# gregc-91/GPU-Raytracing

Hardware: AMD Instinct MI355X
Metric: Mrays/s at 1920x1080 primary rays + BVH build ms, 1M-tri scene (higher is better)
Workload: dtype f32; 1 GPU; grid_mesh(G=708, seed=1) = 1002528 triangles, 1920x1080, 1 spp, camera A (top-down), render_type 0; LBVH replicated per GPU; parallelism=row-bands x1, 8 frames in flight on 8 HIP streams

## Files before the change

### gpu-raytracing_amd/csrc/rt_traverse.hpp

```cpp
#pragma once

#include "rt_device.hpp"
#include "rt_math.h"

namespace rt {

constexpr int kStackLds = 16;
constexpr int kStackMax = 64;
constexpr uint32_t kPrefetchMinPrims = 8u << 20;
#ifndef RT_TRACE_WAVES
#define RT_TRACE_WAVES 4
#endif
constexpr int kTraceWaves = RT_TRACE_WAVES;
#ifndef RT_TRACE_MIN_WAVES
#define RT_TRACE_MIN_WAVES 7
#endif
#ifndef RT_TRACE_LEAN_EXTRA
#define RT_TRACE_LEAN_EXTRA 1
#endif
#ifndef RT_TRACE_PF_WAVES
#define RT_TRACE_PF_WAVES 5
#endif

#ifndef RT_TRACE_UNIFORM_MAX
#define RT_TRACE_UNIFORM_MAX 0
#endif
constexpr int kUniformMax = RT_TRACE_UNIFORM_MAX;
#ifndef RT_TRACE_UNIFORM_STICKY
#define RT_TRACE_UNIFORM_STICKY 1
#endif
constexpr bool kUniformSticky = RT_TRACE_UNIFORM_STICKY != 0;
#ifndef RT_TRACE_PAIR_BARRIER
#define RT_TRACE_PAIR_BARRIER 0
#endif
#ifndef RT_TRACE_LEAF_WIDE
#define RT_TRACE_LEAF_WIDE 1
#endif

constexpr int kParkNum = 8, kParkDen = 1;

#ifndef RT_TRACE_XCD_CHUNK
#define RT_TRACE_XCD_CHUNK 8
#endif
__device__ __forceinline__ uint32_t xcd_chunk_block(uint32_t bid, uint32_t nb)
{
    constexpr uint32_t kXcdChunk = RT_TRACE_XCD_CHUNK;
    const uint32_t full = nb / (8u * kXcdChunk) * (8u * kXcdChunk);
    const uint32_t xcd = bid & 7u, loc = bid >> 3;
    return bid < full ? (loc / kXcdChunk) * (8u * kXcdChunk) + xcd * kXcdChunk + (loc % kXcdChunk) : bid;
}

typedef __attribute__((address_space(3))) uint32_t lds_u32;

struct Ray {
    float ox, oy, oz, dx, dy, dz, ix, iy, iz, tmin, tmax;
};
struct Hit {
    uint32_t primitive_id, tri_id;
    float bu, bv;
};

struct NoFilter {
    static constexpr bool active = false;
};

template <class Filter = NoFilter>
__device__ __forceinline__ bool intersect_tri(float v0x, float v0y, float v0z, float v1x, float v1y, float v1z,
                                              float v2x, float v2y, float v2z, Ray& r, Hit& h, uint32_t tri_id,
                                              uint32_t prim_id, Filter flt = Filter())
{
    const float epsilon = 0.000000001f;
    const float e1x = v1x - v0x, e1y = v1y - v0y, e1z = v1z - v0z;
    const float e2x = v2x - v0x, e2y = v2y - v0y, e2z = v2z - v0z;
    const float hx = r.dy * e2z - r.dz * e2y, hy = r.dz * e2x - r.dx * e2z, hz = r.dx * e2y - r.dy * e2x;
    const float a = e1x * hx + e1y * hy + e1z * hz;
    if (a > -epsilon && a < epsilon) return false;
    const float f = 1.0f / a;
    const float sx = r.ox - v0x, sy = r.oy - v0y, sz = r.oz - v0z;
    const float u = f * (sx * hx + sy * hy + sz * hz);
    if (u < 0.0f || u > 1.0f) return false;
    const float qx = sy * e1z - sz * e1y, qy = sz * e1x - sx * e1z, qz = sx * e1y - sy * e1x;
    const float v = f * (r.dx * qx + r.dy * qy + r.dz * qz);
    if (v < 0.0f || (u + v) > 1.0f) return false;
    const float t = f * (e2x * qx + e2y * qy + e2z * qz);
    if (t < r.tmin || t > r.tmax) return false;
    if constexpr (Filter::active) {
        if (!flt.keep(a, prim_id)) return false;
    }
    r.tmax = t;
    h.primitive_id = prim_id;
    h.tri_id = tri_id;
    h.bu = u;
    h.bv = v;
    return true;
}

enum : uint32_t { PH_STEP = 0, PH_LEAF0 = 1, PH_LEAF1 = 2, PH_DONE = 3 };
constexpr uint32_t kNoNear = 0xFFFFFFFFu;

typedef uint32_t SpillArray[kStackMax - kStackLds];

struct Trav {
    lds_u32* lds;
    uint32_t* spill;
    int sp;
    uint32_t cur;
    uint32_t near_e;
    float near_d;
    uint32_t phase;
    uint32_t leaf;
    float f1, k1;
    uint32_t e1;
    uint32_t t1;
    uint32_t box_tests, tri_tests;
    uint4 pf0, pf1, pf2, pf3;

    __device__ __forceinline__ void push(uint32_t e)
    {
        if (sp < kStackLds) lds[sp * 64] = e;
        else if (sp < kStackMax) spill[sp - kStackLds] = e;
        sp = min(sp + 1, kStackMax);
    }
    __device__ __forceinline__ void inner_hit(bool in, uint32_t e, float front)
    {
        const bool closer = (front < near_d) | ((front == near_d) & ((e & kIndexMask) > (near_e & kIndexMask)));
        if (in & (near_e != kNoNear)) push(closer ? near_e : e);
        const bool take = in & closer;
        near_e = take ? e : near_e;
        near_d = take ? front : near_d;
    }
    __device__ __forceinline__ void advance()
    {
        const uint32_t cnt = cur >> 29;
        if (cnt > 2) { cur = ((cur & kIndexMask) + 2) | ((cnt - 2) << 29); return; }
        const bool keep = (near_e != kNoNear) & (sp < kStackMax);
        if (keep) cur = near_e;
        else if (sp == 0) phase = PH_DONE;
        else { --sp; cur = sp < kStackLds ? lds[sp * 64] : spill[sp - kStackLds]; }
        near_e = kNoNear;
        near_d = __builtin_inff();
    }
    __device__ __forceinline__ void second_slot(float tmin, float tmax)
    {
        const bool valid = t1 != RT_CHILD_NONE;
        const bool hit = valid & (k1 >= f1) & (f1 <= tmax) & (k1 >= tmin);
        box_tests += valid ? 1u : 0u;
        const bool is_leaf = hit & (t1 == RT_CHILD_TRI);
        inner_hit(hit & !is_leaf, e1, f1);
        if (is_leaf) { leaf = e1; phase = PH_LEAF1; }
    }
};

__device__ __forceinline__ void slab(const uint4& a, const uint4& b, const Ray& r, float& front, float& back)
{
    typedef float v2f __attribute__((ext_vector_type(2)));
    const v2f o2 = {r.ox, r.oy}, i2 = {r.ix, r.iy};
    const v2f lo = {__uint_as_float(a.x), __uint_as_float(a.y)}, hi = {__uint_as_float(b.x), __uint_as_float(b.y)};
    const v2f t1 = (lo - o2) * i2, t2 = (hi - o2) * i2;
    const float t1z = (__uint_as_float(a.z) - r.oz) * r.iz, t2z = (__uint_as_float(b.z) - r.oz) * r.iz;
    front = fmaxf(fmaxf(fminf(t1.x, t2.x), fminf(t1.y, t2.y)), fminf(t1z, t2z));
    back = fminf(fminf(fmaxf(t1.x, t2.x), fmaxf(t1.y, t2.y)), fmaxf(t1z, t2z));
}

template <bool PF, class Params>
__device__ __forceinline__ void prefetch_pair(const Params& p, Trav& t)
{
    if constexpr (PF) {
        if (t.phase == PH_STEP) {
            const uint4* np = reinterpret_cast<const uint4*>(p.nodes + (t.cur & kIndexMask));
            const int o1 = (t.cur >> 29) > 1 ? 2 : 0;
            t.pf0 = np[0]; t.pf1 = np[1]; t.pf2 = np[o1]; t.pf3 = np[o1 + 1];
        }
    }
}

template <bool PF, class Params>
__device__ __forceinline__ void box_step_on(const Params& p, const Ray& r, Trav& t, bool two, const uint4& a0, const uint4& b0,
                                            const uint4& a1, const uint4& b1)
{
    float f0, k0;
    slab(a0, b0, r, f0, k0);
    slab(a1, b1, r, t.f1, t.k1);
    t.e1 = (b1.w & kIndexMask) | (a1.w & ~kIndexMask);
    t.t1 = two ? (b1.w >> 29) : (uint32_t)RT_CHILD_NONE;
    const uint32_t type0 = b0.w >> 29;
    const uint32_t e0 = (b0.w & kIndexMask) | (a0.w & ~kIndexMask);
    const bool valid0 = type0 != RT_CHILD_NONE;
    const bool hit0 = valid0 & (k0 >= f0) & (f0 <= r.tmax) & (k0 >= r.tmin);
    t.box_tests += valid0 ? 1u : 0u;
    const bool leaf0 = hit0 & (type0 == RT_CHILD_TRI);
    t.inner_hit(hit0 & !leaf0, e0, f0);
    if (leaf0) { t.leaf = e0; t.phase = PH_LEAF0; }
    else {
        t.second_slot(r.tmin, r.tmax);
        if (t.phase == PH_STEP) { t.advance(); prefetch_pair<PF>(p, t); }
    }
}

template <bool PF, class Params>
__device__ __forceinline__ void box_step(const Params& p, const Ray& r, Trav& t)
{
    const uint32_t cnt = t.cur >> 29;
    const uint4* np = reinterpret_cast<const uint4*>(p.nodes + (t.cur & kIndexMask));
#ifdef RT_EXP_BOX_PAD
#pragma unroll
    for (int q = 0; q < RT_EXP_BOX_PAD; q++) asm volatile("v_mov_b32 %0, %0" : "+v"(t.box_tests));
#endif
    const bool two = cnt > 1;
    const int o1 = two ? 2 : 0;
    uint4 a0, b0, a1, b1;
    if constexpr (PF) { a0 = t.pf0; b0 = t.pf1; a1 = t.pf2; b1 = t.pf3; }
    else {
        a0 = np[0]; b0 = np[1]; a1 = np[o1]; b1 = np[o1 + 1];
#if RT_TRACE_PAIR_BARRIER
        __builtin_amdgcn_sched_barrier(0);
#endif
    }
    box_step_on<PF>(p, r, t, two, a0, b0, a1, b1);
}

typedef uint32_t u32x4 __attribute__((ext_vector_type(4)));
typedef const __attribute__((address_space(4))) u32x4* const_u4_ptr;
template <class Params>
__device__ __forceinline__ void box_step_shared(const Params& p, const Ray& r, Trav& t, uint32_t c)
{
    c = (uint32_t)__builtin_amdgcn_readfirstlane((int)c);
    const const_u4_ptr np = (const_u4_ptr)(uintptr_t)(p.nodes + (c & kIndexMask));
    const bool two = (c >> 29) > 1;
    const int o1 = two ? 2 : 0;
    const u32x4 a0 = np[0], b0 = np[1], a1 = np[o1], b1 = np[o1 + 1];
    box_step_on<false>(p, r, t, two, make_uint4(a0.x, a0.y, a0.z, a0.w), make_uint4(b0.x, b0.y, b0.z, b0.w),
                       make_uint4(a1.x, a1.y, a1.z, a1.w), make_uint4(b1.x, b1.y, b1.z, b1.w));
}

template <bool PF, class Params>
__device__ __forceinline__ bool box_step_wave(const Params& p, const Ray& r, Trav& t, uint64_t st)
{
    if constexpr (!PF && kUniformMax > 0) {
        constexpr int K = kUniformMax > 0 ? kUniformMax : 1;
        uint32_t cs[K];
        uint64_t ms[K];
        uint64_t rest = st;
#pragma unroll
        for (int k = 0; k < kUniformMax; k++) {
            cs[k] = 0; ms[k] = 0;
            if (rest) {
                cs[k] = (uint32_t)__builtin_amdgcn_readlane((int)t.cur, __ffsll((unsigned long long)rest) - 1);
                ms[k] = __builtin_amdgcn_ballot_w64(t.phase == PH_STEP && t.cur == cs[k]);
                rest &= ~ms[k];
            }
        }
        if (rest == 0) {
#pragma unroll
            for (int k = 0; k < kUniformMax; k++)
                if (ms[k]) { if (t.phase == PH_STEP && t.cur == cs[k]) box_step_shared(p, r, t, cs[k]); }
            return true;
        }
    }
    if (t.phase == PH_STEP) box_step<PF>(p, r, t);
    return false;
}

template <bool PF, bool ANY = false, class Params, class Filter = NoFilter>
__device__ __forceinline__ bool trace_ray(const Params& p, Ray& r, Hit& h, Trav& t, bool active, uint32_t* steps,
                                          Filter flt = Filter())
{
    t.sp = 0;
    t.cur = (p.root & kIndexMask) | (p.count << 29);
    t.near_e = kNoNear;
    t.near_d = __builtin_inff();
    t.phase = (active && p.count > 0) ? PH_STEP : PH_DONE;
    t.box_tests = 0;
    t.tri_tests = 0;
    t.t1 = 0;
    t.e1 = 0;
    t.f1 = t.k1 = 0.0f;
    t.leaf = 0;
    prefetch_pair<PF>(p, t);
    bool tri_hit = false;
    uint32_t nbox = 0, nleaf = 0;
    bool shared = true;
#ifdef RT_EXP_UNIFORM_STATS
    uint32_t ustat[4] = {0, 0, 0, 0};
#endif

    while (true) {
        uint64_t stepping, parked;
        while (true) {
            stepping = __builtin_amdgcn_ballot_w64(t.phase == PH_STEP);
            parked = __builtin_amdgcn_ballot_w64((t.phase - 1u) < 2u);
            if (stepping == 0 || __popcll(stepping) * p.park_den < __popcll(parked) * p.park_num) break;
            nbox += 2;
#ifdef RT_EXP_UNIFORM_STATS
            {
                uint64_t rest = stepping;
                int distinct = 0;
                while (rest && distinct < 5) {
                    const int l0 = __ffsll((unsigned long long)rest) - 1;
                    const uint32_t c0 = (uint32_t)__builtin_amdgcn_readlane((int)t.cur, l0);
                    rest &= ~__builtin_amdgcn_ballot_w64(t.phase == PH_STEP && t.cur == c0);
                    distinct++;
                }
                ustat[distinct <= 1 ? 0 : (distinct == 2 ? 1 : (distinct <= 4 ? 2 : 3))]++;
            }
#endif
            if constexpr (!PF && kUniformMax > 0) {
                if (!kUniformSticky || shared) {
                    shared = box_step_wave<PF>(p, r, t, stepping);
                    const uint64_t again = __builtin_amdgcn_ballot_w64(t.phase == PH_STEP);
                    if (again) shared = box_step_wave<PF>(p, r, t, again);
                    continue;
                }
            }
            if (t.phase == PH_STEP) box_step<PF>(p, r, t);
            if (t.phase == PH_STEP) box_step<PF>(p, r, t);
        }
        if ((stepping | parked) == 0) break;
        nleaf++;
        if ((t.phase - 1u) < 2u) {
            t.tri_tests++;
            const uint32_t li = t.leaf & kIndexMask;
            const uint4* tp = reinterpret_cast<const uint4*>(p.leaves + li);
            uint4 l0 = tp[0], l1 = tp[1], l2 = tp[2], l3 = tp[3];
#if RT_TRACE_LEAF_WIDE
            asm volatile("" : "+v"(l0.x), "+v"(l0.y), "+v"(l0.z), "+v"(l0.w), "+v"(l1.x), "+v"(l1.y), "+v"(l1.z), "+v"(l1.w),
                              "+v"(l2.x), "+v"(l2.y), "+v"(l2.z), "+v"(l2.w), "+v"(l3.x), "+v"(l3.y), "+v"(l3.z), "+v"(l3.w));
#endif
            bool hit_tri = intersect_tri(__uint_as_float(l0.x), __uint_as_float(l0.y), __uint_as_float(l0.z),
                                         __uint_as_float(l1.x), __uint_as_float(l1.y), __uint_as_float(l1.z),
                                         __uint_as_float(l2.x), __uint_as_float(l2.y), __uint_as_float(l2.z),
                                         r, h, li << 1, l0.w, flt);
            if ((t.leaf >> 29) > 0 && (l3.x != l2.x || l3.y != l2.y || l3.z != l2.z))
                hit_tri |= intersect_tri(__uint_as_float(l2.x), __uint_as_float(l2.y), __uint_as_float(l2.z),
                                         __uint_as_float(l1.x), __uint_as_float(l1.y), __uint_as_float(l1.z),
                                         __uint_as_float(l3.x), __uint_as_float(l3.y), __uint_as_float(l3.z),
                                         r, h, (li << 1) + 1, l1.w, flt);
            tri_hit |= hit_tri;
            if (ANY && hit_tri) {
                t.phase = PH_DONE;
            } else {
                const bool was_first = t.phase == PH_LEAF0;
                t.phase = PH_STEP;
                if (was_first) t.second_slot(r.tmin, r.tmax);
                if (t.phase == PH_STEP) { t.advance(); prefetch_pair<PF>(p, t); }
            }
        }
    }
#ifdef RT_EXP_UNIFORM_STATS
    steps[0] += ustat[RT_EXP_UNIFORM_STATS == 1 ? 0 : 2];
    steps[1] += ustat[RT_EXP_UNIFORM_STATS == 1 ? 1 : 3];
    (void)nbox; (void)nleaf;
#elif !defined(RT_TRACE_NO_STEPS)
    steps[0] += nbox;
    steps[1] += nleaf;
#endif
    return tri_hit;
}

__device__ __forceinline__ void camera_ray(const rt_camera& cam, uint32_t w, uint32_t h, uint32_t x, uint32_t y, float ox,
                                           float oy, Ray& r)
{
    const float ndcx = 2 * (((float)x + ox) / (float)w) - 1;
    const float ndcy = 2 * (((float)y + oy) / (float)h) - 1;
    const float px = (ndcx * cam.u.x + ndcy * cam.v.x) + 1.0f * cam.w.x;
    const float py = (ndcx * cam.u.y + ndcy * cam.v.y) + 1.0f * cam.w.y;
    const float pz = (ndcx * cam.u.z + ndcy * cam.v.z) + 1.0f * cam.w.z;
    const float inv_len = 1.0f / sqrtf(px * px + py * py + pz * pz);
    r.dx = px * inv_len; r.dy = py * inv_len; r.dz = pz * inv_len;
    r.ox = cam.position.x; r.oy = cam.position.y; r.oz = cam.position.z;
    r.tmin = 0.00001f;
    r.tmax = cam.max_depth;
}

__device__ __forceinline__ void subpixel_offset(uint32_t s, uint32_t spp, float& ox, float& oy)
{
    const uint32_t side = spp == 4 ? 2u : 4u;
    ox = ((float)(s % side) + 0.5f) / (float)side;
    oy = ((float)((s / side) % side) + 0.5f) / (float)side;
}

}
```

### gpu-raytracing_amd/csrc/trace_kernel.hip

```cpp
#include <cstdio>
#include <cstdlib>

#include "rt_device.hpp"
#include "rt_launch.hpp"
#include "rt_math.h"
#include "rt_shade.hpp"
#include "rt_traverse.hpp"

namespace rt {

#ifdef RT_TRACE_TUNING
constexpr int kRenderDebugBoxCount = 100;
#else
constexpr int kRenderDebugBoxCount = -1;
#endif
#ifndef RT_TRACE_TILE_2X2
#define RT_TRACE_TILE_2X2 0
#endif


constexpr uint32_t kCtrSlots = 256, kCtrSub = 16;
struct alignas(64) CtrSlot {
    unsigned long long part[kCtrSub][8];
    unsigned long long top, pad[7];
};
__device__ CtrSlot g_ctr[kCtrSlots];

struct TraceParams {
    const rt_node* nodes;
    const rt_triangle_pair* leaves;
    const rt_attributes* attributes;
    const rt_material* materials;
    const rt_texture* textures;
    const rt_camera* camera;
    float light[3];
    uint32_t root, count, num_materials, num_textures;
    uint8_t* rgba8;
    uint32_t w, h, y0, y1, spp;
    unsigned long long* counters;
    uint32_t tiles_x, num_tiles;
    uint32_t strip_tiles, strip_first, strip_stride;
    int park_num, park_den;
    uint32_t ctr_slot;
};



template <int RENDER, bool PF>
__device__ __forceinline__ void shade_sample(const TraceParams& p, const rt_camera& cam, uint32_t x, uint32_t y,
                                             float ox, float oy, Trav& t, bool active, uint32_t& box_acc,
                                             uint32_t& tri_acc, uint32_t* steps, float& R, float& G, float& B, float& A)
{
    const float max_depth = cam.max_depth;
    Ray r;
    camera_ray(cam, p.w, p.h, x, y, ox, oy, r);
    r.ix = 1.0f / r.dx; r.iy = 1.0f / r.dy; r.iz = 1.0f / r.dz;
    Hit h = {0u, 0u, 0.f, 0.f};
    const bool hit = trace_ray<PF>(p, r, h, t, active, steps);
    const uint32_t box_tests = t.box_tests, tri_tests = t.tri_tests;
    box_acc += box_tests;
    tri_acc += tri_tests;
    const float depth = hit ? r.tmax : 0.0f;
    R = G = B = 0;
    A = 255.0f;

    if (RENDER == RT_RENDER_DEPTH) {
        R = G = B = fminf(1.0f, depth / max_depth) * 255;
        return;
    }
    if (RENDER == RT_RENDER_BOXTESTS) {
        G = B = fminf(box_tests / 180.0f, 1.0f) * 255;
        return;
    }
    if (RENDER == kRenderDebugBoxCount) {
        R = __uint_as_float(box_tests);
        return;
    }
    if (RENDER == RT_RENDER_TRIANGLE_TESTS) {
        const float g = fminf(tri_tests / 32.0f, 1.0f);
        R = g * 100; G = g * 255; B = g * 100;
        return;
    }
    const bool lit = active && hit;
    const bool fetch = active && (hit || RENDER == RT_RENDER_LODS);
    rt_material mat = {};
    Surface s = {};
    int material_id = 0;
    if (fetch) {
        const rt_triangle_pair* pair = p.leaves + (h.tri_id >> 1);
        const bool second = h.tri_id & 1;
        const uint32_t rot = second ? pair->rotations[1] : pair->rotations[0];
        const rt_attributes* at = p.attributes + h.primitive_id;
        const int i0 = rot == 1 ? 2 : (rot == 2 ? 1 : 0);
        const int i1 = rot == 1 ? 0 : (rot == 2 ? 2 : 1);
        const int i2 = rot == 1 ? 1 : (rot == 2 ? 0 : 2);
        material_id = at->material_id;
        mat = p.materials[(uint32_t)material_id < p.num_materials ? (uint32_t)material_id : 0u];
        if ((uint32_t)mat.texture >= p.num_textures) mat.texture = -1;
        if ((uint32_t)mat.bump >= p.num_textures) mat.bump = -1;
        if ((uint32_t)mat.disp >= p.num_textures) mat.disp = -1;
        const rt_float3 n0 = at->normal[i0], n1 = at->normal[i1], n2 = at->normal[i2];
        s.n[0] = v3(n0.x, n0.y, n0.z); s.n[1] = v3(n1.x, n1.y, n1.z); s.n[2] = v3(n2.x, n2.y, n2.z);
        if (render_uses_surface(RENDER)) {
            s.uv[0][0] = at->uv[i0][0]; s.uv[0][1] = at->uv[i0][1];
            s.uv[1][0] = at->uv[i1][0]; s.uv[1][1] = at->uv[i1][1];
            s.uv[2][0] = at->uv[i2][0]; s.uv[2][1] = at->uv[i2][1];
            const rt_float3 a = second ? pair->v2 : pair->v0, b = pair->v1, c = second ? pair->v3 : pair->v2;
            s.tri[0] = v3(a.x, a.y, a.z); s.tri[1] = v3(b.x, b.y, b.z); s.tri[2] = v3(c.x, c.y, c.z);
        }
    }
    const float spread = 2.0f / p.w;
    if (RENDER == RT_RENDER_LODS) {
        if (!active) return;
        if (mat.texture != -1 && hit) {
            const float lod = compute_lod(r, h, spread, s, p.textures[mat.texture]);
            R = G = B = A = (float)(((uint32_t)((int)lod * 20)) & 255u);
        } else {
            R = 255; G = 0; B = 255;
        }
        return;
    }
    if (RENDER == RT_RENDER_MATERIAL_ID) {
        if (lit) hsv_to_rgb255((float)material_id / p.num_materials, 1.0f, 1.0f, R, G, B);
        return;
    }
    if (RENDER == RT_RENDER_TEXTURE) {
        if (!lit) return;
        if (mat.texture != -1) {
            const rt_texture& tex = p.textures[mat.texture];
            const float lod = compute_lod(r, h, spread, s, tex);
            const U8x4 c = trilinear_sample(tex, interp_uv(s, h.bu, h.bv), lod);
            R = (float)c.c[0]; G = (float)c.c[1]; B = (float)c.c[2]; A = (float)c.c[3];
        } else {
            R = mat.diffuse.x * 255; G = mat.diffuse.y * 255; B = mat.diffuse.z * 255;
        }
        return;
    }
    constexpr bool use_textures = RENDER == RT_RENDER_TEXTURE_LIT || RENDER == RT_RENDER_TEXTURE_LIT_SHADOWS;
    constexpr bool use_bump = use_textures;
    constexpr bool use_shadows = RENDER == RT_RENDER_TEXTURE_LIT_SHADOWS;
    const float hx = r.ox + r.dx * r.tmax, hy = r.oy + r.dy * r.tmax, hz = r.oz + r.dz * r.tmax;
    float lx = p.light[0] - hx, ly = p.light[1] - hy, lz = p.light[2] - hz;
    const float to_light = sqrtf(lx * lx + ly * ly + lz * lz);
    const float linv = 1.0f / to_light;
    lx *= linv; ly *= linv; lz *= linv;
    bool shadowed = false;
    if (use_shadows) {
        Ray sr;
        sr.ox = hx; sr.oy = hy; sr.oz = hz;
        sr.dx = lx; sr.dy = ly; sr.dz = lz;
        sr.ix = 1.0f / lx; sr.iy = 1.0f / ly; sr.iz = 1.0f / lz;
        sr.tmin = 0.001f;
        sr.tmax = to_light;
        Hit sh = {0u, 0u, 0.f, 0.f};
        shadowed = trace_ray<PF>(p, sr, sh, t, lit, steps);
    }
    if (!lit) return;
    const float w0 = 1 - h.bu - h.bv;
    V3 n = vadd(vadd(vscale(s.n[0], w0), vscale(s.n[1], h.bu)), vscale(s.n[2], h.bv));
    if (use_bump && mat.disp != -1) {
        const rt_texture& disp = p.textures[mat.disp];
        const float lod = compute_lod(r, h, spread, s, disp);
        V3 tbn[3];
        tangent_matrix(s, tbn);
        const U8x4 smp = trilinear_sample(disp, interp_uv(s, h.bu, h.bv), lod);
        n = v3((float)smp.c[0] / 255.0f, (float)smp.c[1] / 255.0f, (float)smp.c[2] / 255.0f);
        n = vnormalize(v3(n.x * 2.0f - 1.0f, n.y * 2.0f - 1.0f, n.z * 2.0f - 1.0f));
        n = vnormalize(v3(vdot(tbn[0], n), vdot(tbn[1], n), vdot(tbn[2], n)));
    } else if (use_bump && mat.bump != -1) {
        const rt_texture& bump = p.textures[mat.bump];
        const float lod = compute_lod(r, h, spread, s, bump);
        V3 tbn[3];
        tangent_matrix(s, tbn);
        n = bump2normal(bump, tbn, interp_uv(s, h.bu, h.bv), lod);
    }
    const float nx = n.x, ny = n.y, nz = n.z;
    const float lcx = 1.0f, lcy = 0.9f, lcz = 0.8f;
    float dterm = 1.0f * fmaxf(nx * lx + ny * ly + nz * lz, 0.0f);
    const float nlx = -lx, nly = -ly, nlz = -lz;
    const float ndl = nx * nlx + ny * nly + nz * nlz;
    const float rx = nlx - (nx * 2.0f) * ndl, ry = nly - (ny * 2.0f) * ndl, rz = nlz - (nz * 2.0f) * ndl;
    const double sb = fmax((double)((-r.dx) * rx + (-r.dy) * ry + (-r.dz) * rz), 0.0);
    float sp = (float)(1.0f * rt_pow_d(sb, (double)mat.specular_exp));
    float odx = mat.diffuse.x, ody = mat.diffuse.y, odz = mat.diffuse.z;
    if (use_textures && mat.texture != -1) {
        const rt_texture& tex = p.textures[mat.texture];
        const float lod = compute_lod(r, h, spread, s, tex);
        const U8x4 smp = bilinear_sample(tex, interp_uv(s, h.bu, h.bv), (int)lod);
        odx = (float)smp.c[0] / 255; ody = (float)smp.c[1] / 255; odz = (float)smp.c[2] / 255;
    }
    float dfx = lcx * dterm, dfy = lcy * dterm, dfz = lcz * dterm;
    float spx = lcx * sp, spy = lcy * sp, spz = lcz * sp;
    if (shadowed) { dfx = dfy = dfz = 0.0f; spx = spy = spz = 0.0f; }
    const float cr = (dfx * odx + (lcx * 0.2f) * mat.ambient.x) + spx * mat.specular.x;
    const float cg = (dfy * ody + (lcy * 0.2f) * mat.ambient.y) + spy * mat.specular.y;
    const float cb = (dfz * odz + (lcz * 0.2f) * mat.ambient.z) + spz * mat.specular.z;
    R = clampf(cr, 0.0f, 1.0f) * 255;
    G = clampf(cg, 0.0f, 1.0f) * 255;
    B = clampf(cb, 0.0f, 1.0f) * 255;
}

template <int RENDER, bool PF>
__global__ __launch_bounds__(kTraceWaves * 64, PF ? RT_TRACE_PF_WAVES : ((RENDER <= 2 || RENDER == kRenderDebugBoxCount) ? RT_TRACE_MIN_WAVES + RT_TRACE_LEAN_EXTRA : RT_TRACE_MIN_WAVES))
void trace_kernel(TraceParams p)
{
    __shared__ uint32_t stack_lds[kTraceWaves][kStackLds][64];
    __shared__ unsigned long long csum[4];
    __shared__ uint32_t carrive;
    const int lane = threadIdx.x & 63, wave = threadIdx.x >> 6;
    if (p.counters) {
        if (threadIdx.x < 4) csum[threadIdx.x] = 0ull;
        if (threadIdx.x == 4) carrive = 0u;
        __syncthreads();
    }

    const uint32_t vb = xcd_chunk_block(blockIdx.x, gridDim.x);
#if RT_TRACE_TILE_2X2
    const uint32_t blocks_x = (p.tiles_x + 1) / 2;
    const uint32_t tx = (vb % blocks_x) * 2 + (wave & 1), ty = (vb / blocks_x) * 2 + (wave >> 1);
    const uint32_t tile = tx < p.tiles_x ? ty * p.tiles_x + tx : p.num_tiles;
#else
    const uint32_t tile = vb * kTraceWaves + wave;
    const uint32_t tx = tile % p.tiles_x, ty = tile / p.tiles_x;
#endif

    const uint32_t lx = (lane & 1) | ((lane >> 1) & 2) | ((lane >> 2) & 4);
    const uint32_t ly = ((lane >> 1) & 1) | ((lane >> 2) & 2) | ((lane >> 3) & 4);
    const uint32_t x = tx * 8 + lx;
    uint32_t y = p.y0 + ty * 8 + ly, out_y = y;
    if (p.strip_tiles) {
        const uint32_t strip = p.strip_first + (ty / p.strip_tiles) * p.strip_stride;
        y = (strip * p.strip_tiles + ty % p.strip_tiles) * 8 + ly;
        out_y = ty * 8 + ly;
    }
    const bool active = tile < p.num_tiles && x < p.w && y < p.y1;

    const rt_camera cam = *p.camera;
    SpillArray spill;
    Trav t;
    t.lds = (lds_u32*)&stack_lds[wave][0][lane];
    t.spill = spill;
    uint32_t box_acc = 0, tri_acc = 0;
    uint32_t steps[2] = {0u, 0u};
    float R, G, B, A;
    if (p.spp <= 1) {
        shade_sample<RENDER, PF>(p, cam, x, y, 0.5f, 0.5f, t, active, box_acc, tri_acc, steps, R, G, B, A);
    } else {
        float ar = 0, ag = 0, ab = 0, aa = 0;
        const uint32_t side = p.spp == 4 ? 2u : 4u;
        for (uint32_t s = 0; s < p.spp; s++) {
            const float ox = ((float)(s % side) + 0.5f) / (float)side, oy = ((float)((s / side) % side) + 0.5f) / (float)side;
            shade_sample<RENDER, PF>(p, cam, x, y, ox, oy, t, active, box_acc, tri_acc, steps, R, G, B, A);
            ar += R; ag += G; ab += B; aa += A;
        }
        R = ar / (float)p.spp; G = ag / (float)p.spp; B = ab / (float)p.spp; A = aa / (float)p.spp;
    }
    if (active) {
        uint32_t px = sat_u8(R) | (sat_u8(G) << 8) | (sat_u8(B) << 16) | (sat_u8(A) << 24);
        if (RENDER == kRenderDebugBoxCount) px = __float_as_uint(R);
        reinterpret_cast<uint32_t*>(p.rgba8)[(size_t)out_y * p.w + x] = px;
    }
    if (p.counters) {
        const uint32_t bsum = wave_sum_u32(box_acc), tsum = wave_sum_u32(tri_acc);
        uint32_t last = 0;
        if (lane == 0) {
            atomicAdd(&csum[0], (unsigned long long)bsum);
            atomicAdd(&csum[1], (unsigned long long)tsum);
            atomicAdd(&csum[2], (unsigned long long)steps[0]);
            atomicAdd(&csum[3], (unsigned long long)steps[1]);
            __builtin_amdgcn_fence(__ATOMIC_RELEASE, "workgroup");
            last = atomicAdd(&carrive, 1u) == (uint32_t)kTraceWaves - 1u ? 1u : 0u;
            __builtin_amdgcn_fence(__ATOMIC_ACQUIRE, "workgroup");
        }
        if (__builtin_amdgcn_readfirstlane((int)last)) {
            CtrSlot& S = g_ctr[p.ctr_slot];
            const uint32_t sub = blockIdx.x % kCtrSub;
            if (lane < 4) {
                const unsigned long long v = *(volatile unsigned long long*)&csum[lane];
                const unsigned long long old = v ? __hip_atomic_fetch_add(&S.part[sub][lane], v, __ATOMIC_RELAXED, __HIP_MEMORY_SCOPE_AGENT) : 0ull;
                asm volatile("" ::"v"((uint32_t)old), "v"((uint32_t)(old >> 32)) : "memory");
            }
            uint32_t fin = 0;
            if (lane == 0) {
                const uint32_t members = (gridDim.x - sub + kCtrSub - 1) / kCtrSub;
                if (__hip_atomic_fetch_add(&S.part[sub][4], 1ull, __ATOMIC_RELAXED, __HIP_MEMORY_SCOPE_AGENT) + 1ull == members) {
                    const uint32_t rows = min(gridDim.x, kCtrSub);
                    fin = __hip_atomic_fetch_add(&S.top, 1ull, __ATOMIC_RELAXED, __HIP_MEMORY_SCOPE_AGENT) + 1ull == rows ? 1u : 0u;
                }
            }
            if (__builtin_amdgcn_readfirstlane((int)fin)) {
                __builtin_amdgcn_fence(__ATOMIC_ACQUIRE, "agent");
                unsigned long long* cell = &S.part[lane >> 2][lane & 3];
                unsigned long long v = __hip_atomic_load(cell, __ATOMIC_RELAXED, __HIP_MEMORY_SCOPE_AGENT);
                __hip_atomic_store(cell, 0ull, __ATOMIC_RELAXED, __HIP_MEMORY_SCOPE_AGENT);
                if (lane < (int)kCtrSub) __hip_atomic_store(&S.part[lane][4], 0ull, __ATOMIC_RELAXED, __HIP_MEMORY_SCOPE_AGENT);
                if (lane == 0) __hip_atomic_store(&S.top, 0ull, __ATOMIC_RELAXED, __HIP_MEMORY_SCOPE_AGENT);
#pragma unroll
                for (int off = 4; off < 64; off <<= 1) v += __shfl_xor(v, off, 64);
                if (lane < 4 && v) atomicAdd(&p.counters[lane], v);
            }
        }
    }
}

hipError_t launch_trace(const TraceLaunch& t, hipStream_t st)
{
    if (t.y1 <= t.y0 || t.w == 0) return hipSuccess;
    TraceParams p;
    p.nodes = t.as.nodes;
    p.leaves = t.as.triangles;
    p.attributes = t.scene.attributes;
    p.materials = t.scene.materials;
    p.textures = t.scene.textures;
    p.camera = t.scene.camera;
    p.light[0] = t.scene.light[0]; p.light[1] = t.scene.light[1]; p.light[2] = t.scene.light[2];
    p.root = t.as.root;
    p.count = t.as.count;
    p.num_materials = t.scene.num_materials;
    p.num_textures = t.scene.textures ? t.scene.num_textures : 0;
    p.rgba8 = t.rgba8;
    p.w = t.w; p.h = t.h; p.y0 = t.y0; p.y1 = t.y1; p.spp = t.spp;
    p.counters = reinterpret_cast<unsigned long long*>(t.counters);
    static std::atomic<uint32_t> ctr_seq{0};
    p.ctr_slot = t.counters ? ctr_seq.fetch_add(1u, std::memory_order_relaxed) % kCtrSlots : 0u;
    p.tiles_x = (t.w + 7) / 8;
    uint32_t tiles_y = (t.y1 - t.y0 + 7) / 8;
    p.strip_tiles = t.strip_rows / 8;
    p.strip_first = t.strip_first;
    p.strip_stride = t.strip_stride;
    if (p.strip_tiles) {
        const uint32_t nstrips = (t.h + t.strip_rows - 1) / t.strip_rows;
        if (t.strip_first >= nstrips) return hipSuccess;
        tiles_y = ((nstrips - t.strip_first + t.strip_stride - 1) / t.strip_stride) * p.strip_tiles;
    }
    p.num_tiles = p.tiles_x * tiles_y;
    p.park_num = kParkNum;
    p.park_den = kParkDen;
#ifdef RT_TRACE_TUNING
    static const int* park = [] {
        static int v[2] = {kParkNum, kParkDen};
        if (const char* e = getenv("RT_TRACE_PARK")) {
            int a = 0, b = 0;
            if (sscanf(e, "%d,%d", &a, &b) == 2 && a > 0 && b > 0) { v[0] = a; v[1] = b; }
        }
        return v;
    }();
    p.park_num = park[0];
    p.park_den = park[1];
#endif
#if RT_TRACE_TILE_2X2
    static_assert(kTraceWaves == 4, "a 2 x 2 block of tiles per workgroup");
    const uint32_t blocks = ((p.tiles_x + 1) / 2) * ((tiles_y + 1) / 2);
#else
    const uint32_t blocks = (p.num_tiles + kTraceWaves - 1) / kTraceWaves;
#endif
    const dim3 grid(blocks), block(kTraceWaves * 64);
    const bool pf = t.scene.num_attributes >= kPrefetchMinPrims;
#define RT_TRACE_CASE(R) case R: if (pf) trace_kernel<R, true><<<grid, block, 0, st>>>(p); else trace_kernel<R, false><<<grid, block, 0, st>>>(p); break;
    switch (t.render_type) {
    RT_TRACE_CASE(RT_RENDER_DEPTH)
    RT_TRACE_CASE(RT_RENDER_BOXTESTS)
    RT_TRACE_CASE(RT_RENDER_TRIANGLE_TESTS)
    RT_TRACE_CASE(RT_RENDER_MATERIAL_ID)
    RT_TRACE_CASE(RT_RENDER_DIFFUSE)
    RT_TRACE_CASE(RT_RENDER_LODS)
    RT_TRACE_CASE(RT_RENDER_TEXTURE)
    RT_TRACE_CASE(RT_RENDER_TEXTURE_LIT)
    RT_TRACE_CASE(RT_RENDER_TEXTURE_LIT_SHADOWS)
#ifdef RT_TRACE_TUNING
    case kRenderDebugBoxCount: trace_kernel<kRenderDebugBoxCount, false><<<grid, block, 0, st>>>(p); break;
#endif
    default: return hipErrorInvalidValue;
    }
#undef RT_TRACE_CASE
    return hipGetLastError();
}

}
```

Measured before the change: 1118 Mrays/s.

## Hold popped lanes until quad neighbours reach the same stack node

Adds a quad-wait mode for primary-ray traversal. A lane that just popped a node from its LDS stack checks, through DPP quad broadcasts and one 16-byte LDS read of its quad's stack slots, whether a neighbour with a deeper stack holds the same node, and if so holds off stepping. The aim is to re-converge adjacent rays onto shared nodes so the quad fetches the same node data and SIMD divergence drops. In exchange each step carries extra DPP, LDS and compare work, and held lanes idle. The path is on by default for non-prefetch depth and box/triangle-test renders with a BVH root count of at least two.

```diff
diff --git a/gpu-raytracing_amd/csrc/rt_traverse.hpp b/gpu-raytracing_amd/csrc/rt_traverse.hpp
--- a/gpu-raytracing_amd/csrc/rt_traverse.hpp
+++ b/gpu-raytracing_amd/csrc/rt_traverse.hpp
@@ -95,7 +95,15 @@
     return true;
 }
 
-enum : uint32_t { PH_STEP = 0, PH_LEAF0 = 1, PH_LEAF1 = 2, PH_DONE = 3 };
+#ifndef RT_TRACE_QUAD_WAIT
+#define RT_TRACE_QUAD_WAIT 1
+#endif
+
+#ifndef RT_TRACE_QUAD_WAIT_SECOND
+#define RT_TRACE_QUAD_WAIT_SECOND 0
+#endif
+
+enum : uint32_t { PH_STEP = 0, PH_LEAF0 = 1, PH_LEAF1 = 2, PH_DONE = 3, PH_STEP_POP = 4 };
 constexpr uint32_t kNoNear = 0xFFFFFFFFu;
 
 typedef uint32_t SpillArray[kStackMax - kStackLds];
@@ -129,6 +137,7 @@
         near_e = take ? e : near_e;
         near_d = take ? front : near_d;
     }
+    template <bool QW = false>
     __device__ __forceinline__ void advance()
     {
         const uint32_t cnt = cur >> 29;
@@ -136,7 +145,10 @@
         const bool keep = (near_e != kNoNear) & (sp < kStackMax);
         if (keep) cur = near_e;
         else if (sp == 0) phase = PH_DONE;
-        else { --sp; cur = sp < kStackLds ? lds[sp * 64] : spill[sp - kStackLds]; }
+        else {
+            --sp; cur = sp < kStackLds ? lds[sp * 64] : spill[sp - kStackLds];
+            if constexpr (QW) phase = PH_STEP_POP;
+        }
         near_e = kNoNear;
         near_d = __builtin_inff();
     }
@@ -174,10 +186,11 @@
     }
 }
 
-template <bool PF, class Params>
+template <bool PF, bool QW = false, class Params>
 __device__ __forceinline__ void box_step_on(const Params& p, const Ray& r, Trav& t, bool two, const uint4& a0, const uint4& b0,
                                             const uint4& a1, const uint4& b1)
 {
+    if constexpr (QW) t.phase = PH_STEP;
     float f0, k0;
     slab(a0, b0, r, f0, k0);
     slab(a1, b1, r, t.f1, t.k1);
@@ -193,11 +206,11 @@
     if (leaf0) { t.leaf = e0; t.phase = PH_LEAF0; }
     else {
         t.second_slot(r.tmin, r.tmax);
-        if (t.phase == PH_STEP) { t.advance(); prefetch_pair<PF>(p, t); }
-    }
-}
-
-template <bool PF, class Params>
+        if (t.phase == PH_STEP) { t.template advance<QW>(); prefetch_pair<PF>(p, t); }
+    }
+}
+
+template <bool PF, bool QW = false, class Params>
 __device__ __forceinline__ void box_step(const Params& p, const Ray& r, Trav& t)
 {
     const uint32_t cnt = t.cur >> 29;
@@ -216,7 +229,25 @@
         __builtin_amdgcn_sched_barrier(0);
 #endif
     }
-    box_step_on<PF>(p, r, t, two, a0, b0, a1, b1);
+    box_step_on<PF, QW>(p, r, t, two, a0, b0, a1, b1);
+}
+
+template <bool ANY>
+__device__ __forceinline__ bool quad_hold(const Trav& t)
+{
+    const bool popped = t.phase == PH_STEP_POP && t.sp < kStackLds;
+    const int key = ANY && t.phase == PH_DONE ? 0 : t.sp;
+    const int k0 = __builtin_amdgcn_mov_dpp(key, 0x00, 0xF, 0xF, true), k1 = __builtin_amdgcn_mov_dpp(key, 0x55, 0xF, 0xF, true);
+    const int k2 = __builtin_amdgcn_mov_dpp(key, 0xAA, 0xF, 0xF, true), k3 = __builtin_amdgcn_mov_dpp(key, 0xFF, 0xF, 0xF, true);
+    bool hold = false;
+    if (popped) {
+        typedef uint32_t lds_u32x4 __attribute__((ext_vector_type(4)));
+        typedef __attribute__((address_space(3))) lds_u32x4 lds_quad;
+        const lds_u32x4 e = *(const lds_quad*)(((uintptr_t)t.lds & ~(uintptr_t)15) + (uintptr_t)t.sp * 256u);
+        hold = ((k0 > t.sp) & (e.x == t.cur)) | ((k1 > t.sp) & (e.y == t.cur)) | ((k2 > t.sp) & (e.z == t.cur)) |
+               ((k3 > t.sp) & (e.w == t.cur));
+    }
+    return hold;
 }
 
 typedef uint32_t u32x4 __attribute__((ext_vector_type(4)));
@@ -261,10 +292,11 @@
     return false;
 }
 
-template <bool PF, bool ANY = false, class Params, class Filter = NoFilter>
+template <bool PF, bool ANY = false, bool QW = false, class Params, class Filter = NoFilter>
 __device__ __forceinline__ bool trace_ray(const Params& p, Ray& r, Hit& h, Trav& t, bool active, uint32_t* steps,
                                           Filter flt = Filter())
 {
+    static_assert(!(PF && QW), "prefetch_pair tests phase == PH_STEP: a PH_STEP_POP lane would step on a stale prefetched pair");
     t.sp = 0;
     t.cur = (p.root & kIndexMask) | (p.count << 29);
     t.near_e = kNoNear;
@@ -287,6 +319,20 @@
     while (true) {
         uint64_t stepping, parked;
         while (true) {
+            if constexpr (QW) {
+                const bool go = ((t.phase & 3u) == PH_STEP) & !quad_hold<ANY>(t);
+                stepping = __builtin_amdgcn_ballot_w64(go);
+                parked = __builtin_amdgcn_ballot_w64((t.phase - 1u) < 2u);
+                if (stepping == 0 || __popcll(stepping) * p.park_den < __popcll(parked) * p.park_num) break;
+                nbox += 2;
+                if (go) box_step<PF, true>(p, r, t);
+#if RT_TRACE_QUAD_WAIT_SECOND
+                if (((t.phase & 3u) == PH_STEP) & !quad_hold<ANY>(t)) box_step<PF, true>(p, r, t);
+#else
+                if ((t.phase & 3u) == PH_STEP) box_step<PF, true>(p, r, t);
+#endif
+                continue;
+            }
             stepping = __builtin_amdgcn_ballot_w64(t.phase == PH_STEP);
             parked = __builtin_amdgcn_ballot_w64((t.phase - 1u) < 2u);
             if (stepping == 0 || __popcll(stepping) * p.park_den < __popcll(parked) * p.park_num) break;
@@ -342,7 +388,7 @@
                 const bool was_first = t.phase == PH_LEAF0;
                 t.phase = PH_STEP;
                 if (was_first) t.second_slot(r.tmin, r.tmax);
-                if (t.phase == PH_STEP) { t.advance(); prefetch_pair<PF>(p, t); }
+                if (t.phase == PH_STEP) { t.template advance<QW>(); prefetch_pair<PF>(p, t); }
             }
         }
     }
diff --git a/gpu-raytracing_amd/csrc/trace_kernel.hip b/gpu-raytracing_amd/csrc/trace_kernel.hip
--- a/gpu-raytracing_amd/csrc/trace_kernel.hip
+++ b/gpu-raytracing_amd/csrc/trace_kernel.hip
@@ -46,7 +46,12 @@
 
 
 
-template <int RENDER, bool PF>
+constexpr bool trace_quad_wait(int render, bool pf)
+{
+    return !pf && (RT_TRACE_QUAD_WAIT >= 2 || (RT_TRACE_QUAD_WAIT == 1 && (render <= 2 || render == kRenderDebugBoxCount)));
+}
+
+template <int RENDER, bool PF, bool QW>
 __device__ __forceinline__ void shade_sample(const TraceParams& p, const rt_camera& cam, uint32_t x, uint32_t y,
                                              float ox, float oy, Trav& t, bool active, uint32_t& box_acc,
                                              uint32_t& tri_acc, uint32_t* steps, float& R, float& G, float& B, float& A)
@@ -56,7 +61,7 @@
     camera_ray(cam, p.w, p.h, x, y, ox, oy, r);
     r.ix = 1.0f / r.dx; r.iy = 1.0f / r.dy; r.iz = 1.0f / r.dz;
     Hit h = {0u, 0u, 0.f, 0.f};
-    const bool hit = trace_ray<PF>(p, r, h, t, active, steps);
+    const bool hit = trace_ray<PF, false, QW>(p, r, h, t, active, steps);
     const uint32_t box_tests = t.box_tests, tri_tests = t.tri_tests;
     box_acc += box_tests;
     tri_acc += tri_tests;
@@ -153,7 +158,7 @@
         sr.tmin = 0.001f;
         sr.tmax = to_light;
         Hit sh = {0u, 0u, 0.f, 0.f};
-        shadowed = trace_ray<PF>(p, sr, sh, t, lit, steps);
+        shadowed = trace_ray<PF, false, QW>(p, sr, sh, t, lit, steps);
     }
     if (!lit) return;
     const float w0 = 1 - h.bu - h.bv;
@@ -200,11 +205,11 @@
     B = clampf(cb, 0.0f, 1.0f) * 255;
 }
 
-template <int RENDER, bool PF>
+template <int RENDER, bool PF, bool QW = false>
 __global__ __launch_bounds__(kTraceWaves * 64, PF ? RT_TRACE_PF_WAVES : ((RENDER <= 2 || RENDER == kRenderDebugBoxCount) ? RT_TRACE_MIN_WAVES + RT_TRACE_LEAN_EXTRA : RT_TRACE_MIN_WAVES))
 void trace_kernel(TraceParams p)
 {
-    __shared__ uint32_t stack_lds[kTraceWaves][kStackLds][64];
+    __shared__ __attribute__((aligned(16))) uint32_t stack_lds[kTraceWaves][kStackLds][64];
     __shared__ unsigned long long csum[4];
     __shared__ uint32_t carrive;
     const int lane = threadIdx.x & 63, wave = threadIdx.x >> 6;
@@ -244,13 +249,13 @@
     uint32_t steps[2] = {0u, 0u};
     float R, G, B, A;
     if (p.spp <= 1) {
-        shade_sample<RENDER, PF>(p, cam, x, y, 0.5f, 0.5f, t, active, box_acc, tri_acc, steps, R, G, B, A);
+        shade_sample<RENDER, PF, QW>(p, cam, x, y, 0.5f, 0.5f, t, active, box_acc, tri_acc, steps, R, G, B, A);
     } else {
         float ar = 0, ag = 0, ab = 0, aa = 0;
         const uint32_t side = p.spp == 4 ? 2u : 4u;
         for (uint32_t s = 0; s < p.spp; s++) {
             const float ox = ((float)(s % side) + 0.5f) / (float)side, oy = ((float)((s / side) % side) + 0.5f) / (float)side;
-            shade_sample<RENDER, PF>(p, cam, x, y, ox, oy, t, active, box_acc, tri_acc, steps, R, G, B, A);
+            shade_sample<RENDER, PF, QW>(p, cam, x, y, ox, oy, t, active, box_acc, tri_acc, steps, R, G, B, A);
             ar += R; ag += G; ab += B; aa += A;
         }
         R = ar / (float)p.spp; G = ag / (float)p.spp; B = ab / (float)p.spp; A = aa / (float)p.spp;
@@ -356,7 +361,12 @@
 #endif
     const dim3 grid(blocks), block(kTraceWaves * 64);
     const bool pf = t.scene.num_attributes >= kPrefetchMinPrims;
-#define RT_TRACE_CASE(R) case R: if (pf) trace_kernel<R, true><<<grid, block, 0, st>>>(p); else trace_kernel<R, false><<<grid, block, 0, st>>>(p); break;
+    const bool qw = t.as.count >= 2;
+#define RT_TRACE_CASE(R) case R: \
+        if (pf) trace_kernel<R, true><<<grid, block, 0, st>>>(p); \
+        else if (trace_quad_wait(R, false) && qw) trace_kernel<R, false, trace_quad_wait(R, false)><<<grid, block, 0, st>>>(p); \
+        else trace_kernel<R, false><<<grid, block, 0, st>>>(p); \
+        break;
     switch (t.render_type) {
     RT_TRACE_CASE(RT_RENDER_DEPTH)
     RT_TRACE_CASE(RT_RENDER_BOXTESTS)
```

Result: faster. 1175 Mrays/s (median of 6 runs) (+5.0%).
